# JoeyYoung/adapcc

Hardware: AMD Instinct MI355X
Metric: gpt2_ddp_tokens_per_sec (higher is better)
Workload: dtype bf16; 1 GPU; model=gpt2-small-124M, global_batch=128, seq_len=1024, parallelism=dp1, bucket_cap_mb=100, hipgraph=True, precision=bf16, transport=native

## Files before the change

### adapcc_amd/models/gpt2.py

```python

from __future__ import annotations

import math
from dataclasses import dataclass

import torch
import torch.nn as nn
import torch.nn.functional as F

from ..ops.fused import FusedLayerNorm


@dataclass
class GPT2Config:
    vocab_size: int = 50257
    n_positions: int = 1024
    n_embd: int = 768
    n_layer: int = 12
    n_head: int = 12
    dropout: float = 0.0

    @classmethod
    def small(cls) -> "GPT2Config":
        return cls()

    @classmethod
    def tiny(cls) -> "GPT2Config":
        return cls(vocab_size=2048, n_positions=256, n_embd=128, n_layer=2,
                   n_head=4)

    @classmethod
    def medium(cls) -> "GPT2Config":
        return cls(n_embd=1024, n_layer=24, n_head=16)


class CausalSelfAttention(nn.Module):
    def __init__(self, cfg: GPT2Config):
        super().__init__()
        assert cfg.n_embd % cfg.n_head == 0
        self.n_head = cfg.n_head
        self.c_attn = nn.Linear(cfg.n_embd, 3 * cfg.n_embd)
        self.c_proj = nn.Linear(cfg.n_embd, cfg.n_embd)
        self.dropout = cfg.dropout

    def forward(self, x: torch.Tensor) -> torch.Tensor:
        B, T, C = x.shape
        qkv = self.c_attn(x)
        q, k, v = qkv.split(C, dim=2)
        hd = C // self.n_head
        q = q.view(B, T, self.n_head, hd).transpose(1, 2)
        k = k.view(B, T, self.n_head, hd).transpose(1, 2)
        v = v.view(B, T, self.n_head, hd).transpose(1, 2)
        from ..ops.attention import flash_attention

        y = flash_attention(
            q, k, v, causal=True,
            dropout_p=self.dropout if self.training else 0.0,
        )
        y = y.transpose(1, 2).contiguous().view(B, T, C)
        return self.c_proj(y)


class MLP(nn.Module):
    def __init__(self, cfg: GPT2Config):
        super().__init__()
        self.c_fc = nn.Linear(cfg.n_embd, 4 * cfg.n_embd)
        self.c_proj = nn.Linear(4 * cfg.n_embd, cfg.n_embd)

    def forward(self, x: torch.Tensor) -> torch.Tensor:
        from ..ops.fused import fused_gelu

        return self.c_proj(fused_gelu(self.c_fc(x)))


class Block(nn.Module):
    def __init__(self, cfg: GPT2Config):
        super().__init__()
        self.ln_1 = FusedLayerNorm(cfg.n_embd)
        self.attn = CausalSelfAttention(cfg)
        self.ln_2 = FusedLayerNorm(cfg.n_embd)
        self.mlp = MLP(cfg)

    def forward(self, x: torch.Tensor) -> torch.Tensor:
        x = x + self.attn(self.ln_1(x))
        x = x + self.mlp(self.ln_2(x))
        return x


class GPT2(nn.Module):
    def __init__(self, cfg: GPT2Config):
        super().__init__()
        self.cfg = cfg
        self.wte = nn.Embedding(cfg.vocab_size, cfg.n_embd)
        self.wpe = nn.Embedding(cfg.n_positions, cfg.n_embd)
        self.drop = nn.Dropout(cfg.dropout)
        self.h = nn.ModuleList(Block(cfg) for _ in range(cfg.n_layer))
        self.ln_f = FusedLayerNorm(cfg.n_embd)
        self.lm_head = nn.Linear(cfg.n_embd, cfg.vocab_size, bias=False)
        self.lm_head.weight = self.wte.weight
        self.apply(self._init)
        for name, p in self.named_parameters():
            if name.endswith("c_proj.weight"):
                nn.init.normal_(p, mean=0.0,
                                std=0.02 / math.sqrt(2 * cfg.n_layer))

    @staticmethod
    def _init(m: nn.Module) -> None:
        if isinstance(m, nn.Linear):
            nn.init.normal_(m.weight, mean=0.0, std=0.02)
            if m.bias is not None:
                nn.init.zeros_(m.bias)
        elif isinstance(m, nn.Embedding):
            nn.init.normal_(m.weight, mean=0.0, std=0.02)

    def num_params(self, non_embedding: bool = True) -> int:
        n = sum(p.numel() for p in self.parameters())
        if non_embedding:
            n -= self.wpe.weight.numel()
        return n

    def forward(self, idx: torch.Tensor, targets: torch.Tensor = None):
        B, T = idx.shape
        pos = torch.arange(T, device=idx.device)
        x = self.drop(self.wte(idx) + self.wpe(pos))
        for block in self.h:
            x = block(x)
        x = self.ln_f(x)
        logits = self.lm_head(x)
        loss = None
        if targets is not None:
            from ..ops.fused import fused_cross_entropy

            loss = fused_cross_entropy(
                logits.view(-1, logits.size(-1)), targets.view(-1)
            )
        return logits, loss
```

### adapcc_amd/ops/attention.py

```python

from __future__ import annotations

import math

import torch

from .fused import _core

__all__ = ["flash_attention", "fa_supported"]


def _strides3(t: torch.Tensor):
    return [t.stride(0), t.stride(1), t.stride(2)]


def _row_ok(t: torch.Tensor) -> bool:
    if t.stride(3) != 1:
        return False
    if t.data_ptr() % 16 != 0:
        return False
    return all(s % 8 == 0 for s in _strides3(t))


def fa_supported(q: torch.Tensor, k: torch.Tensor, v: torch.Tensor,
                 causal: bool, dropout_p: float) -> bool:
    if not (causal and dropout_p == 0.0):
        return False
    if not (q.is_cuda and q.dtype == torch.bfloat16):
        return False
    if q.dim() != 4 or q.shape != k.shape or q.shape != v.shape:
        return False
    B, H, S, D = q.shape
    if D != 64 or S % 128 != 0 or S < 128:
        return False
    if not (_row_ok(q) and _row_ok(k) and _row_ok(v)):
        return False
    return bool(_core())


class _FlashAttnFn(torch.autograd.Function):
    @staticmethod
    def forward(ctx, q, k, v, scale):
        c = _core()
        B, H, S, D = q.shape
        o = torch.empty((B, H, S, D), dtype=q.dtype, device=q.device)
        lse = torch.empty((B, H, S), dtype=torch.float32, device=q.device)
        strides = _strides3(q) + _strides3(k) + _strides3(v) + _strides3(o)
        stream = torch.cuda.current_stream(q.device).cuda_stream
        c.fa_fwd(q.data_ptr(), k.data_ptr(), v.data_ptr(), o.data_ptr(),
                 lse.data_ptr(), B, H, S, strides, scale, stream)
        ctx.save_for_backward(q, k, v, o, lse)
        ctx.scale = scale
        return o

    @staticmethod
    def backward(ctx, dout):
        c = _core()
        q, k, v, o, lse = ctx.saved_tensors
        B, H, S, D = q.shape
        do = dout.contiguous()
        delta = (do.float() * o.float()).sum(-1)
        dq = torch.empty((B, H, S, D), dtype=q.dtype, device=q.device)
        dk = torch.empty_like(dq)
        dv = torch.empty_like(dq)
        strides = (_strides3(q) + _strides3(k) + _strides3(v) +
                   _strides3(do) + _strides3(dq) + _strides3(dk) +
                   _strides3(dv))
        stream = torch.cuda.current_stream(q.device).cuda_stream
        c.fa_bwd(q.data_ptr(), k.data_ptr(), v.data_ptr(), do.data_ptr(),
                 lse.data_ptr(), delta.data_ptr(), dq.data_ptr(),
                 dk.data_ptr(), dv.data_ptr(), B, H, S, strides, ctx.scale,
                 stream)
        return dq, dk, dv, None


def flash_attention(q: torch.Tensor, k: torch.Tensor, v: torch.Tensor,
                    causal: bool = True, dropout_p: float = 0.0,
                    scale: float = None) -> torch.Tensor:
    if fa_supported(q, k, v, causal, dropout_p):
        s = scale if scale is not None else 1.0 / math.sqrt(q.shape[-1])
        return _FlashAttnFn.apply(q, k, v, s)
    return torch.nn.functional.scaled_dot_product_attention(
        q, k, v, is_causal=causal, dropout_p=dropout_p, scale=scale)
```

### adapcc_amd/ops/csrc/attn.hip

```cpp

#include <hip/hip_runtime.h>
#include <hip/hip_bf16.h>

#include <cstdint>
#include <stdexcept>
#include <string>

namespace adapcc {

namespace {

typedef __attribute__((ext_vector_type(8))) __bf16 bf16x8;
typedef __attribute__((ext_vector_type(4))) __bf16 bf16x4;
typedef __attribute__((ext_vector_type(16))) float f32x16;

constexpr int kQT = 128;
constexpr float kNegBig = -3.0e38f;
constexpr float kLog2e = 1.4426950408889634f;
constexpr float kLn2 = 0.6931471805599453f;

__device__ __forceinline__ f32x16 mfma(bf16x8 a, bf16x8 b, f32x16 c) {
  return __builtin_amdgcn_mfma_f32_32x32x16_bf16(a, b, c, 0, 0, 0);
}

// ... 91 lines not shown

  const int qb = qt * kQT + wave * 32;
  const int qrow = qb + (lane & 31);

  bf16x8 qf[4];
#pragma unroll
  for (int c = 0; c < 4; ++c)
    qf[c] = *reinterpret_cast<const bf16x8*>(
        qg + (long)qrow * p.qs.ss + c * 16 + hi * 8);

  f32x16 acc0 = {}, acc1 = {};
  float m = kNegBig, ssum = 0.f;
  const float c1 = p.scale * kLog2e;
  float mc = m * c1;
  const float thr = 8.0f / p.scale;

  const int srow = threadIdx.x >> 3;
  const int scol = (threadIdx.x & 7) * 8;
  const int n64 = (qt + 1) * (kQT / 64);

  {
    *reinterpret_cast<uint4*>(kimg(0) + row_img_byte(srow, scol)) =
        *reinterpret_cast<const uint4*>(kg + (long)srow * p.ks.ss + scol);
    *reinterpret_cast<uint4*>(kimg(0) + 4096 + row_img_byte(srow, scol)) =
        *reinterpret_cast<const uint4*>(kg + (long)(srow + 32) * p.ks.ss +
                                        scol);
    *reinterpret_cast<uint4*>(vimg(0) + row_img_byte(srow, scol)) =
        *reinterpret_cast<const uint4*>(vg + (long)srow * p.vs.ss + scol);
    *reinterpret_cast<uint4*>(vimg(0) + 4096 + row_img_byte(srow, scol)) =
        *reinterpret_cast<const uint4*>(vg + (long)(srow + 32) * p.vs.ss +
                                        scol);
  }
  __syncthreads();

  int cur = 0;
  for (int t = 0; t < n64; ++t) {
    uint4 nk0, nk1, nv0, nv1;
    const bool pref = t + 1 < n64;
    if (pref) {
      const long kb0 = (long)(t + 1) * 64 + srow;
      nk0 = *reinterpret_cast<const uint4*>(kg + kb0 * p.ks.ss + scol);
      nk1 = *reinterpret_cast<const uint4*>(kg + (kb0 + 32) * p.ks.ss + scol);
      nv0 = *reinterpret_cast<const uint4*>(vg + kb0 * p.vs.ss + scol);
      nv1 = *reinterpret_cast<const uint4*>(vg + (kb0 + 32) * p.vs.ss + scol);
    }

#pragma unroll
    for (int half = 0; half < 2; ++half) {
      const int kbase = t * 64 + half * 32;
      if (kbase > qb + 31) break;
      const char* ki = kimg(cur) + half * 4096;
      const char* vi = vimg(cur) + half * 4096;

      f32x16 s = {};
      __builtin_amdgcn_s_setprio(1);
#pragma unroll
      for (int c = 0; c < 4; ++c)
        s = mfma(read_row_frag(ki, lane, c), qf[c], s);
      __builtin_amdgcn_s_setprio(0);

      float pv[16];
      float tmax = kNegBig;
      if (kbase + 31 > qb) {
#pragma unroll
        for (int r = 0; r < 16; ++r) {
          const int kglob = kbase + crow(r, hi);
          pv[r] = (kglob > qrow) ? kNegBig : s[r];
          tmax = fmaxf(tmax, pv[r]);
        }
      } else {
#pragma unroll
        for (int r = 0; r < 16; ++r) {
          pv[r] = s[r];
          tmax = fmaxf(tmax, pv[r]);
        }
      }
      tmax = fmaxf(tmax, __shfl_xor(tmax, 32, 64));
      if (!__all(tmax <= m + thr)) {
        const float mnew = fmaxf(m, tmax);
        const float alpha = __builtin_amdgcn_exp2f((m - mnew) * c1);
        m = mnew;
        mc = m * c1;
        ssum *= alpha;
#pragma unroll
        for (int r = 0; r < 16; ++r) {
          acc0[r] *= alpha;
          acc1[r] *= alpha;
        }
      }

      float psum = 0.f;
#pragma unroll
      for (int r = 0; r < 16; ++r) {
        pv[r] = __builtin_amdgcn_exp2f(__builtin_fmaf(pv[r], c1, -mc));
        psum += pv[r];
      }
      ssum += psum;

      const bf16x8 p0 = pack_frag(&pv[0]);
      const bf16x8 p1 = pack_frag(&pv[8]);

      __builtin_amdgcn_s_setprio(1);
      acc0 = mfma(read_tr_frag(vi, lane, 0, 0), p0, acc0);
      acc0 = mfma(read_tr_frag(vi, lane, 1, 0), p1, acc0);
      acc1 = mfma(read_tr_frag(vi, lane, 0, 1), p0, acc1);
      acc1 = mfma(read_tr_frag(vi, lane, 1, 1), p1, acc1);
      __builtin_amdgcn_s_setprio(0);
    }

    if (pref) {
      *reinterpret_cast<uint4*>(kimg(cur ^ 1) + row_img_byte(srow, scol)) =
          nk0;
      *reinterpret_cast<uint4*>(kimg(cur ^ 1) + 4096 +
                                row_img_byte(srow, scol)) = nk1;
      *reinterpret_cast<uint4*>(vimg(cur ^ 1) + row_img_byte(srow, scol)) =
          nv0;
      *reinterpret_cast<uint4*>(vimg(cur ^ 1) + 4096 +
                                row_img_byte(srow, scol)) = nv1;
    }
    __syncthreads();
    cur ^= 1;
  }

  const float stot = ssum + __shfl_xor(ssum, 32, 64);
  const float inv = 1.f / stot;
  if ((lane >> 5) == 0)
    lseg[qrow] = p.scale * m + __builtin_amdgcn_logf(stot) * kLn2;

  __bf16* orow = og + (long)qrow * p.os.ss;
#pragma unroll
  for (int db = 0; db < 2; ++db) {
    const f32x16& a = db ? acc1 : acc0;
#pragma unroll
    for (int mq = 0; mq < 4; ++mq) {
      const int d0 = db * 32 + 8 * mq + 4 * hi;
      unsigned lo, hi2;
      asm("v_cvt_pk_bf16_f32 %0, %2, %3\n\t"
          "v_cvt_pk_bf16_f32 %1, %4, %5"
          : "=&v"(lo), "=&v"(hi2)
          : "v"(a[4 * mq] * inv), "v"(a[4 * mq + 1] * inv),
            "v"(a[4 * mq + 2] * inv), "v"(a[4 * mq + 3] * inv));
      uint2 st = {lo, hi2};
      *reinterpret_cast<uint2*>(orow + d0) = st;
    }
  }
}
#undef kimg
#undef vimg

struct FaBwdParams {
  const __bf16* q;
  const __bf16* k;
  const __bf16* v;
  const __bf16* dout;
  const float* lse;
  const float* delta;
  __bf16* dq;
  __bf16* dk;
  __bf16* dv;
  TStride qs, ks, vs, dos_, dqs, dks, dvs;
  int H, S;
  float scale;
};

__global__ __launch_bounds__(256, 3) void fa_bwd_dq_kernel(FaBwdParams p) {
  __shared__ __attribute__((aligned(16))) char smem[4 * 8192];
#define kimg(i) (smem + (i) * 8192)
#define vimg(i) (smem + 16384 + (i) * 8192)

  const int lane = threadIdx.x & 63;
  const int wave = threadIdx.x >> 6;
  const int hi = lane >> 5;
  const int qt = blockIdx.x;
  const int bh = blockIdx.y;
  const int b = bh / p.H, h = bh % p.H;

  const __bf16* qg = p.q + (long)b * p.qs.sb + (long)h * p.qs.sh;
  const __bf16* kg = p.k + (long)b * p.ks.sb + (long)h * p.ks.sh;
  const __bf16* vg = p.v + (long)b * p.vs.sb + (long)h * p.vs.sh;
  const __bf16* dog = p.dout + (long)b * p.dos_.sb + (long)h * p.dos_.sh;
  __bf16* dqg = p.dq + (long)b * p.dqs.sb + (long)h * p.dqs.sh;

  const int qb = qt * kQT + wave * 32;
  const int qrow = qb + (lane & 31);

  bf16x8 qf[4], dof[4];
#pragma unroll
  for (int c = 0; c < 4; ++c) {
    qf[c] = *reinterpret_cast<const bf16x8*>(
        qg + (long)qrow * p.qs.ss + c * 16 + hi * 8);
    dof[c] = *reinterpret_cast<const bf16x8*>(
        dog + (long)qrow * p.dos_.ss + c * 16 + hi * 8);
  }
  const float lse2 = p.lse[(long)bh * p.S + qrow] * kLog2e;
  const float dvq = p.delta[(long)bh * p.S + qrow];
  const float c1 = p.scale * kLog2e;

  f32x16 dacc0 = {}, dacc1 = {};

  const int srow = threadIdx.x >> 3;
  const int scol = (threadIdx.x & 7) * 8;
  const int n64 = (qt + 1) * (kQT / 64);
  {
    *reinterpret_cast<uint4*>(kimg(0) + row_img_byte(srow, scol)) =
        *reinterpret_cast<const uint4*>(kg + (long)srow * p.ks.ss + scol);
    *reinterpret_cast<uint4*>(kimg(0) + 4096 + row_img_byte(srow, scol)) =
        *reinterpret_cast<const uint4*>(kg + (long)(srow + 32) * p.ks.ss +
                                        scol);
    *reinterpret_cast<uint4*>(vimg(0) + row_img_byte(srow, scol)) =
        *reinterpret_cast<const uint4*>(vg + (long)srow * p.vs.ss + scol);
    *reinterpret_cast<uint4*>(vimg(0) + 4096 + row_img_byte(srow, scol)) =
        *reinterpret_cast<const uint4*>(vg + (long)(srow + 32) * p.vs.ss +
                                        scol);
  }
  __syncthreads();

  int cur = 0;
  for (int t = 0; t < n64; ++t) {
    uint4 nk0, nk1, nv0, nv1;
    const bool pref = t + 1 < n64;
    if (pref) {
      const long kb0 = (long)(t + 1) * 64 + srow;
      nk0 = *reinterpret_cast<const uint4*>(kg + kb0 * p.ks.ss + scol);
      nk1 = *reinterpret_cast<const uint4*>(kg + (kb0 + 32) * p.ks.ss + scol);
      nv0 = *reinterpret_cast<const uint4*>(vg + kb0 * p.vs.ss + scol);
      nv1 = *reinterpret_cast<const uint4*>(vg + (kb0 + 32) * p.vs.ss + scol);
    }

#pragma unroll
    for (int half = 0; half < 2; ++half) {
      const int kbase = t * 64 + half * 32;
      if (kbase > qb + 31) break;
      const char* ki = kimg(cur) + half * 4096;
      const char* vi = vimg(cur) + half * 4096;

      f32x16 s = {}, dp = {};
      __builtin_amdgcn_s_setprio(1);
#pragma unroll
      for (int c = 0; c < 4; ++c) {
        s = mfma(read_row_frag(ki, lane, c), qf[c], s);
        dp = mfma(read_row_frag(vi, lane, c), dof[c], dp);
      }
      __builtin_amdgcn_s_setprio(0);

      float ds[16];
      if (kbase + 31 > qb) {
#pragma unroll
        for (int r = 0; r < 16; ++r) {
          const int kglob = kbase + crow(r, hi);
          const float pe =
              (kglob > qrow)
                  ? 0.f
                  : __builtin_amdgcn_exp2f(__builtin_fmaf(s[r], c1, -lse2));
          ds[r] = pe * (dp[r] - dvq) * p.scale;
        }
      } else {
#pragma unroll
        for (int r = 0; r < 16; ++r) {
          const float pe =
              __builtin_amdgcn_exp2f(__builtin_fmaf(s[r], c1, -lse2));
          ds[r] = pe * (dp[r] - dvq) * p.scale;
        }
      }
      const bf16x8 d0 = pack_frag(&ds[0]);
      const bf16x8 d1 = pack_frag(&ds[8]);
      __builtin_amdgcn_s_setprio(1);
      dacc0 = mfma(read_tr_frag(ki, lane, 0, 0), d0, dacc0);
      dacc0 = mfma(read_tr_frag(ki, lane, 1, 0), d1, dacc0);
      dacc1 = mfma(read_tr_frag(ki, lane, 0, 1), d0, dacc1);
      dacc1 = mfma(read_tr_frag(ki, lane, 1, 1), d1, dacc1);
      __builtin_amdgcn_s_setprio(0);
    }

    if (pref) {
      *reinterpret_cast<uint4*>(kimg(cur ^ 1) + row_img_byte(srow, scol)) =
          nk0;
      *reinterpret_cast<uint4*>(kimg(cur ^ 1) + 4096 +
                                row_img_byte(srow, scol)) = nk1;
      *reinterpret_cast<uint4*>(vimg(cur ^ 1) + row_img_byte(srow, scol)) =
          nv0;
      *reinterpret_cast<uint4*>(vimg(cur ^ 1) + 4096 +
                                row_img_byte(srow, scol)) = nv1;
    }
    __syncthreads();
    cur ^= 1;
  }

  __bf16* drow = dqg + (long)qrow * p.dqs.ss;
#pragma unroll
  for (int db = 0; db < 2; ++db) {
    const f32x16& a = db ? dacc1 : dacc0;
#pragma unroll
    for (int mq = 0; mq < 4; ++mq) {
      const int d0 = db * 32 + 8 * mq + 4 * hi;
      unsigned lo, hi2;
      asm("v_cvt_pk_bf16_f32 %0, %2, %3\n\t"
          "v_cvt_pk_bf16_f32 %1, %4, %5"
          : "=&v"(lo), "=&v"(hi2)
          : "v"(a[4 * mq]), "v"(a[4 * mq + 1]), "v"(a[4 * mq + 2]),
            "v"(a[4 * mq + 3]));
      uint2 st = {lo, hi2};
      *reinterpret_cast<uint2*>(drow + d0) = st;
    }
  }
}
#undef kimg
#undef vimg


__global__ __launch_bounds__(256, 2) void fa_bwd_dkv_kernel(FaBwdParams p) {
  __shared__ __attribute__((aligned(16))) char smem[4 * 8192 + 1024];
#define qimg(i) (smem + (i) * 8192)
#define doimg(i) (smem + 16384 + (i) * 8192)
#define lsetile (reinterpret_cast<float*>(smem + 32768))
#define dtile (reinterpret_cast<float*>(smem + 32768 + 512))

  const int lane = threadIdx.x & 63;
  const int wave = threadIdx.x >> 6;
  const int hi = lane >> 5;
  const int kt = blockIdx.x;
  const int bh = blockIdx.y;
  const int b = bh / p.H, h = bh % p.H;

  const __bf16* qg = p.q + (long)b * p.qs.sb + (long)h * p.qs.sh;
  const __bf16* kg = p.k + (long)b * p.ks.sb + (long)h * p.ks.sh;
  const __bf16* vg = p.v + (long)b * p.vs.sb + (long)h * p.vs.sh;
  const __bf16* dog = p.dout + (long)b * p.dos_.sb + (long)h * p.dos_.sh;
  __bf16* dkg = p.dk + (long)b * p.dks.sb + (long)h * p.dks.sh;
  __bf16* dvg = p.dv + (long)b * p.dvs.sb + (long)h * p.dvs.sh;
  const float* lseg = p.lse + (long)bh * p.S;
  const float* deltag = p.delta + (long)bh * p.S;

  const int kbb = kt * kQT + wave * 32;
  const int krow = kbb + (lane & 31);

  bf16x8 kf[4], vf[4];
#pragma unroll
  for (int c = 0; c < 4; ++c) {
    kf[c] = *reinterpret_cast<const bf16x8*>(
        kg + (long)krow * p.ks.ss + c * 16 + hi * 8);
    vf[c] = *reinterpret_cast<const bf16x8*>(
        vg + (long)krow * p.vs.ss + c * 16 + hi * 8);
  }

  const float c1 = p.scale * kLog2e;
  f32x16 dvacc0 = {}, dvacc1 = {}, dkacc0 = {}, dkacc1 = {};

  const int srow = threadIdx.x >> 3;
// ... 78 lines not shown
          const float pe = __builtin_amdgcn_exp2f(
              __builtin_fmaf(sacc[r], c1, -lsec[crow(r, hi)]));
          pv[r] = pe;
          ds[r] = pe * (dp[r] - dc[crow(r, hi)]) * p.scale;
        }
      }
      const bf16x8 p0 = pack_frag(&pv[0]);
      const bf16x8 p1 = pack_frag(&pv[8]);
      __builtin_amdgcn_s_setprio(1);
      dvacc0 = mfma(p0, read_tr_frag(di, lane, 0, 0), dvacc0);
      dvacc0 = mfma(p1, read_tr_frag(di, lane, 1, 0), dvacc0);
      dvacc1 = mfma(p0, read_tr_frag(di, lane, 0, 1), dvacc1);
      dvacc1 = mfma(p1, read_tr_frag(di, lane, 1, 1), dvacc1);
      __builtin_amdgcn_s_setprio(0);
      const bf16x8 e0 = pack_frag(&ds[0]);
      const bf16x8 e1 = pack_frag(&ds[8]);
      __builtin_amdgcn_s_setprio(1);
      dkacc0 = mfma(e0, read_tr_frag(qi, lane, 0, 0), dkacc0);
      dkacc0 = mfma(e1, read_tr_frag(qi, lane, 1, 0), dkacc0);
      dkacc1 = mfma(e0, read_tr_frag(qi, lane, 0, 1), dkacc1);
      dkacc1 = mfma(e1, read_tr_frag(qi, lane, 1, 1), dkacc1);
      __builtin_amdgcn_s_setprio(0);
    }

    if (pref) {
      *reinterpret_cast<uint4*>(qimg(cur ^ 1) + row_img_byte(srow, scol)) =
          nq0;
      *reinterpret_cast<uint4*>(qimg(cur ^ 1) + 4096 +
                                row_img_byte(srow, scol)) = nq1;
      *reinterpret_cast<uint4*>(doimg(cur ^ 1) + row_img_byte(srow, scol)) =
          nd0;
      *reinterpret_cast<uint4*>(doimg(cur ^ 1) + 4096 +
                                row_img_byte(srow, scol)) = nd1;
      if (threadIdx.x < 64) {
        lsetile[((cur ^ 1) ? 64 : 0) + threadIdx.x] = nlse;
        dtile[((cur ^ 1) ? 64 : 0) + threadIdx.x] = ndel;
      }
    }
    __syncthreads();
    cur ^= 1;
  }

  __syncthreads();
  float* scratch = reinterpret_cast<float*>(smem) + wave * 2048;
#pragma unroll
  for (int t = 0; t < 2; ++t) {
    const f32x16& a0 = t ? dkacc0 : dvacc0;
    const f32x16& a1 = t ? dkacc1 : dvacc1;
#pragma unroll
    for (int r = 0; r < 16; ++r) {
      scratch[crow(r, hi) * 64 + (lane & 31)] = a0[r];
      scratch[crow(r, hi) * 64 + 32 + (lane & 31)] = a1[r];
    }
    __builtin_amdgcn_s_waitcnt(0);
    __bf16* outg = (t ? dkg : dvg);
    const TStride& os = t ? p.dks : p.dvs;
    const int row = lane >> 1;
    const int dhalf = (lane & 1) * 32;
#pragma unroll
    for (int mq = 0; mq < 8; ++mq) {
      const float* src = scratch + row * 64 + dhalf + mq * 4;
      unsigned lo, hi2;
      asm("v_cvt_pk_bf16_f32 %0, %2, %3\n\t"
          "v_cvt_pk_bf16_f32 %1, %4, %5"
          : "=&v"(lo), "=&v"(hi2)
          : "v"(src[0]), "v"(src[1]), "v"(src[2]), "v"(src[3]));
      uint2 st = {lo, hi2};
      *reinterpret_cast<uint2*>(outg + (long)(kbb + row) * os.ss + dhalf +
                                mq * 4) = st;
    }
    __syncthreads();
  }
}
#undef qimg
#undef doimg
#undef lsetile
#undef dtile

__global__ void tr_probe_kernel(float* out, int kb, int db) {
  __shared__ __attribute__((aligned(16))) char img[4096];
  const int lane = threadIdx.x & 63;
  for (int i = threadIdx.x; i < 2048; i += 64) {
    const int k = i / 64, d = i % 64;
    *reinterpret_cast<__bf16*>(img + row_img_byte(k, d)) =
        (__bf16)(float)(k * 64 + d);
  }
  __syncthreads();
  bf16x8 f = read_tr_frag(img, lane, kb, db);
  union {
    bf16x8 v;
    __bf16 e[8];
  } u;
  u.v = f;
#pragma unroll
  for (int e = 0; e < 8; ++e) out[lane * 8 + e] = (float)u.e[e];
}

__global__ void pack_probe_kernel(float* out) {
  const int lane = threadIdx.x & 63;
  float p[8];
#pragma unroll
  for (int r = 0; r < 8; ++r) p[r] = (float)(lane * 100 + r);
  bf16x8 f = pack_frag(p);
  union {
    bf16x8 v;
    __bf16 e[8];
  } u;
  u.v = f;
#pragma unroll
  for (int e = 0; e < 8; ++e) out[lane * 8 + e] = (float)u.e[e];
}

__global__ void mfma_probe_kernel(const __bf16* a, const __bf16* b, float* c) {
  const int lane = threadIdx.x & 63;
  union {
    __bf16 e[8];
    bf16x8 f;
  } af, bf;
#pragma unroll
  for (int e = 0; e < 8; ++e) {
    af.e[e] = a[(lane % 32) * 16 + 8 * (lane / 32) + e];
    bf.e[e] = b[(8 * (lane / 32) + e) * 32 + (lane % 32)];
  }
  f32x16 acc = {};
  acc = mfma(af.f, bf.f, acc);
#pragma unroll
  for (int r = 0; r < 16; ++r)
    c[crow(r, lane >> 5) * 32 + (lane % 32)] = acc[r];
}

}

void fa_forward(const void* q, const void* k, const void* v, void* o,
                float* lse, int B, int H, int S, const long* strides,
                float scale, hipStream_t stream) {
  if (S % kQT != 0) throw std::runtime_error("fa_forward: S % 128 != 0");
  FaParams p;
  p.q = (const __bf16*)q;
  p.k = (const __bf16*)k;
  p.v = (const __bf16*)v;
  p.o = (__bf16*)o;
  p.lse = lse;
  p.qs = {strides[0], strides[1], strides[2]};
  p.ks = {strides[3], strides[4], strides[5]};
  p.vs = {strides[6], strides[7], strides[8]};
  p.os = {strides[9], strides[10], strides[11]};
  p.H = H;
  p.S = S;
  p.scale = scale;
  dim3 grid(S / kQT, B * H);
  hipLaunchKernelGGL(fa_fwd_kernel, grid, dim3(256), 0, stream, p);
}

void fa_backward(const void* q, const void* k, const void* v, const void* do_,
                 const float* lse, const float* delta, void* dq, void* dk,
                 void* dv, int B, int H, int S, const long* strides,
                 float scale, hipStream_t stream) {
  if (S % kQT != 0) throw std::runtime_error("fa_backward: S % 128 != 0");
  FaBwdParams p;
  p.q = (const __bf16*)q;
  p.k = (const __bf16*)k;
  p.v = (const __bf16*)v;
  p.dout = (const __bf16*)do_;
  p.lse = lse;
  p.delta = delta;
  p.dq = (__bf16*)dq;
  p.dk = (__bf16*)dk;
  p.dv = (__bf16*)dv;
  p.qs = {strides[0], strides[1], strides[2]};
  p.ks = {strides[3], strides[4], strides[5]};
  p.vs = {strides[6], strides[7], strides[8]};
  p.dos_ = {strides[9], strides[10], strides[11]};
  p.dqs = {strides[12], strides[13], strides[14]};
  p.dks = {strides[15], strides[16], strides[17]};
  p.dvs = {strides[18], strides[19], strides[20]};
  p.H = H;
  p.S = S;
  p.scale = scale;
  dim3 grid(S / kQT, B * H);
  hipLaunchKernelGGL(fa_bwd_dq_kernel, grid, dim3(256), 0, stream, p);
  hipLaunchKernelGGL(fa_bwd_dkv_kernel, grid, dim3(256), 0, stream, p);
}

void mfma_probe(const void* a, const void* b, float* c, hipStream_t stream) {
  hipLaunchKernelGGL(mfma_probe_kernel, dim3(1), dim3(64), 0, stream,
                     (const __bf16*)a, (const __bf16*)b, c);
}

void tr_probe(float* out, int kb, int db, hipStream_t stream) {
  hipLaunchKernelGGL(tr_probe_kernel, dim3(1), dim3(64), 0, stream, out, kb,
                     db);
}

void pack_probe(float* out, hipStream_t stream) {
  hipLaunchKernelGGL(pack_probe_kernel, dim3(1), dim3(64), 0, stream, out);
}

}
```

### adapcc_amd/ops/csrc/bindings.hip

```cpp

#include <pybind11/pybind11.h>
#include <pybind11/stl.h>

#include "common.h"
#include "engine.h"
#include "plan.h"

namespace py = pybind11;
using adapcc::Engine;

static py::dict plan_to_dict(const adapcc::PlanData& p) {
  py::list cs, rs, bs;
  for (const auto& u : p.cunits) {
    py::dict d;
    d["tree"] = u.tree; d["chunk"] = u.chunk;
    d["offset"] = u.offset_elems; d["count"] = u.count_elems;
    d["flag_space"] = (int)u.flag_space;
    py::list nl;
    for (int i = 0; i < u.nnotify; ++i) nl.append(u.notify_rank[i]);
    d["notify_to"] = nl;
    cs.append(d);
  }
  for (const auto& u : p.runits) {
    py::dict d;
    d["tree"] = u.tree; d["chunk"] = u.chunk;
    d["offset"] = u.offset_elems; d["count"] = u.count_elems;
    py::list srcs;
    for (int s = 0; s < u.nsrc; ++s)
      srcs.append(py::make_tuple(u.src_rank[s], (int)u.src_kind[s]));
    d["srcs"] = srcs;
    d["include_self"] = (bool)u.include_self;
    d["notify"] = (bool)u.notify_parent; d["consumer"] = u.parent_rank;
    d["is_root"] = (bool)u.is_root;
    py::list kids;
    for (int c = 0; c < u.nchildren; ++c) kids.append(u.child_rank[c]);
    d["publish_to"] = kids;
    rs.append(d);
  }
  for (const auto& u : p.bunits) {
    py::dict d;
    d["tree"] = u.tree; d["chunk"] = u.chunk;
    d["src_offset"] = u.src_offset_elems; d["dst_offset"] = u.dst_offset_elems;
    d["count"] = u.count_elems;
    d["parent"] = u.parent_rank; d["parent_kind"] = (int)u.parent_kind;
    d["forward"] = (bool)u.forward;
    py::list kids;
    for (int c = 0; c < u.nchildren; ++c) kids.append(u.child_rank[c]);
    d["publish_to"] = kids;
    bs.append(d);
  }
  py::dict out;
  out["copy"] = cs;
  out["reduce"] = rs;
  out["bcast"] = bs;
  out["chunk_elems"] = p.chunk_elems;
  return out;
}

namespace adapcc {
void launch_local_reduce(Dtype dt, void* dst, const void* const* srcs_dev,
                         int nsrc, long count, RedOp op, float scale,
                         hipStream_t stream);
bool ln_supported_api(long cols, int dtype);
void ln_forward(int dtype, const void* x, const void* w, const void* b,
                void* y, float* mean, float* rstd, long rows, long cols,
                float eps, hipStream_t stream);
void ln_backward(int dtype, const void* dy, const void* x, const void* w,
                 const float* mean, const float* rstd, void* dx,
                 float* ws_gamma, float* ws_beta, long rows, long cols,
                 int nblocks, hipStream_t stream);
void ce_forward(int dtype, const void* logits, const void* targets,
                float* loss, float* lse, long rows, long cols,
                long ignore_index, hipStream_t stream);
void ce_backward(int dtype, const void* logits, const void* targets,
                 const float* lse, const float* gscale, void* dlogits,
                 long rows, long cols, long ignore_index, hipStream_t stream);
void fa_forward(const void* q, const void* k, const void* v, void* o,
                float* lse, int B, int H, int S, const long* strides,
                float scale, hipStream_t stream);
void fa_backward(const void* q, const void* k, const void* v, const void* do_,
                 const float* lse, const float* delta, void* dq, void* dk,
                 void* dv, int B, int H, int S, const long* strides,
                 float scale, hipStream_t stream);
void mfma_probe(const void* a, const void* b, float* c, hipStream_t stream);
void gelu_forward(int dtype, const void* x, void* y, long n,
                  hipStream_t stream);
void gelu_backward(int dtype, const void* x, const void* dy, void* dx, long n,
                   hipStream_t stream);
void tr_probe(float* out, int kb, int db, hipStream_t stream);
void pack_probe(float* out, hipStream_t stream);
}

PYBIND11_MODULE(_core, m) {
  m.doc() = "adapcc_amd native engine (MI355X / gfx950)";

  m.def("local_reduce",
        [](uintptr_t dst, const std::vector<uintptr_t>& srcs, long count,
           int dtype, int op, float scale, uintptr_t stream) {
          if (srcs.empty()) throw std::runtime_error("no sources");
          void** d_srcs = nullptr;
          hipError_t e = hipMalloc(&d_srcs, srcs.size() * sizeof(void*));
          if (e != hipSuccess) throw std::runtime_error(hipGetErrorString(e));
          e = hipMemcpy(d_srcs, srcs.data(), srcs.size() * sizeof(void*),
                        hipMemcpyHostToDevice);
          if (e != hipSuccess) throw std::runtime_error(hipGetErrorString(e));
          adapcc::launch_local_reduce(
              (adapcc::Dtype)dtype, reinterpret_cast<void*>(dst),
              (const void* const*)d_srcs, (int)srcs.size(), count,
              (adapcc::RedOp)op, scale, reinterpret_cast<hipStream_t>(stream));
          e = hipGetLastError();
          if (e != hipSuccess) throw std::runtime_error(hipGetErrorString(e));
          e = hipStreamSynchronize(reinterpret_cast<hipStream_t>(stream));
          (void)hipFree(d_srcs);
          if (e != hipSuccess) throw std::runtime_error(hipGetErrorString(e));
        },
        py::arg("dst"), py::arg("srcs"), py::arg("count"), py::arg("dtype"),
        py::arg("op"), py::arg("scale") = 1.0f, py::arg("stream") = 0);

  m.def("ln_supported", &adapcc::ln_supported_api, py::arg("cols"),
        py::arg("dtype"));
  m.def("ln_fwd",
        [](int dtype, uintptr_t x, uintptr_t w, uintptr_t b, uintptr_t y,
           uintptr_t mean, uintptr_t rstd, long rows, long cols, float eps,
           uintptr_t stream) {
          adapcc::ln_forward(dtype, (const void*)x, (const void*)w,
                             (const void*)b, (void*)y, (float*)mean,
                             (float*)rstd, rows, cols, eps,
                             reinterpret_cast<hipStream_t>(stream));
          hipError_t e = hipGetLastError();
          if (e != hipSuccess) throw std::runtime_error(hipGetErrorString(e));
        });
  m.def("ln_bwd",
        [](int dtype, uintptr_t dy, uintptr_t x, uintptr_t w, uintptr_t mean,
           uintptr_t rstd, uintptr_t dx, uintptr_t wsg, uintptr_t wsb,
           long rows, long cols, int nblocks, uintptr_t stream) {
          adapcc::ln_backward(dtype, (const void*)dy, (const void*)x,
                              (const void*)w, (const float*)mean,
                              (const float*)rstd, (void*)dx, (float*)wsg,
                              (float*)wsb, rows, cols, nblocks,
                              reinterpret_cast<hipStream_t>(stream));
          hipError_t e = hipGetLastError();
          if (e != hipSuccess) throw std::runtime_error(hipGetErrorString(e));
        });

  m.def("ce_fwd",
        [](int dtype, uintptr_t logits, uintptr_t targets, uintptr_t loss,
           uintptr_t lse, long rows, long cols, long ignore_index,
           uintptr_t stream) {
          adapcc::ce_forward(dtype, (const void*)logits,
                             (const void*)targets, (float*)loss, (float*)lse,
                             rows, cols, ignore_index,
                             reinterpret_cast<hipStream_t>(stream));
          hipError_t e = hipGetLastError();
          if (e != hipSuccess) throw std::runtime_error(hipGetErrorString(e));
        });
  m.def("ce_bwd",
        [](int dtype, uintptr_t logits, uintptr_t targets, uintptr_t lse,
           uintptr_t gscale, uintptr_t dlogits, long rows, long cols,
           long ignore_index, uintptr_t stream) {
          adapcc::ce_backward(dtype, (const void*)logits,
                              (const void*)targets, (const float*)lse,
                              (const float*)gscale, (void*)dlogits, rows,
                              cols, ignore_index,
                              reinterpret_cast<hipStream_t>(stream));
          hipError_t e = hipGetLastError();
          if (e != hipSuccess) throw std::runtime_error(hipGetErrorString(e));
        });

  m.def("fa_fwd",
        [](uintptr_t q, uintptr_t k, uintptr_t v, uintptr_t o, uintptr_t lse,
           int B, int H, int S, const std::vector<long>& strides, float scale,
           uintptr_t stream) {
          if (strides.size() != 12)
            throw std::runtime_error("fa_fwd: need 12 strides");
          adapcc::fa_forward((const void*)q, (const void*)k, (const void*)v,
                             (void*)o, (float*)lse, B, H, S, strides.data(),
                             scale, reinterpret_cast<hipStream_t>(stream));
          hipError_t e = hipGetLastError();
          if (e != hipSuccess) throw std::runtime_error(hipGetErrorString(e));
        });
  m.def("fa_bwd",
        [](uintptr_t q, uintptr_t k, uintptr_t v, uintptr_t dout,
           uintptr_t lse, uintptr_t delta, uintptr_t dq, uintptr_t dk,
           uintptr_t dv, int B, int H, int S, const std::vector<long>& strides,
           float scale, uintptr_t stream) {
          if (strides.size() != 21)
            throw std::runtime_error("fa_bwd: need 21 strides");
          adapcc::fa_backward((const void*)q, (const void*)k, (const void*)v,
                              (const void*)dout, (const float*)lse,
                              (const float*)delta, (void*)dq, (void*)dk,
                              (void*)dv, B, H, S, strides.data(), scale,
                              reinterpret_cast<hipStream_t>(stream));
          hipError_t e = hipGetLastError();
          if (e != hipSuccess) throw std::runtime_error(hipGetErrorString(e));
        });
  m.def("mfma_probe",
        [](uintptr_t a, uintptr_t b, uintptr_t c, uintptr_t stream) {
          adapcc::mfma_probe((const void*)a, (const void*)b, (float*)c,
                             reinterpret_cast<hipStream_t>(stream));
          hipError_t e = hipGetLastError();
          if (e != hipSuccess) throw std::runtime_error(hipGetErrorString(e));
        });

  m.def("gelu_fwd",
        [](int dtype, uintptr_t x, uintptr_t y, long n, uintptr_t stream) {
          adapcc::gelu_forward(dtype, (const void*)x, (void*)y, n,
                               reinterpret_cast<hipStream_t>(stream));
          hipError_t e = hipGetLastError();
          if (e != hipSuccess) throw std::runtime_error(hipGetErrorString(e));
        });
  m.def("gelu_bwd",
        [](int dtype, uintptr_t x, uintptr_t dy, uintptr_t dx, long n,
           uintptr_t stream) {
          adapcc::gelu_backward(dtype, (const void*)x, (const void*)dy,
                                (void*)dx, n,
                                reinterpret_cast<hipStream_t>(stream));
          hipError_t e = hipGetLastError();
          if (e != hipSuccess) throw std::runtime_error(hipGetErrorString(e));
        });

  m.def("tr_probe",
        [](uintptr_t out, int kb, int db, uintptr_t stream) {
          adapcc::tr_probe((float*)out, kb, db,
                           reinterpret_cast<hipStream_t>(stream));
          hipError_t e = hipGetLastError();
          if (e != hipSuccess) throw std::runtime_error(hipGetErrorString(e));
        });
  m.def("pack_probe",
        [](uintptr_t out, uintptr_t stream) {
          adapcc::pack_probe((float*)out,
                             reinterpret_cast<hipStream_t>(stream));
          hipError_t e = hipGetLastError();
          if (e != hipSuccess) throw std::runtime_error(hipGetErrorString(e));
        });

  m.def("compute_plan",
        [](const std::vector<std::vector<int>>& parents, int rank,
           long total_elems, int esize, long chunk_bytes,
           const std::vector<int>& active,
           const std::vector<double>& slice_weights) {
          auto shape = adapcc::TreeShape::derive(parents);
          uint64_t mask = 0;
          for (int r : active) mask |= (1ull << r);
          if (active.empty()) mask = (1ull << shape.world) - 1;
          return plan_to_dict(adapcc::build_plan(shape, rank, total_elems,
                                                 esize, chunk_bytes, mask,
                                                 slice_weights));
        },
        py::arg("parents"), py::arg("rank"), py::arg("total_elems"),
        py::arg("esize"), py::arg("chunk_bytes"),
        py::arg("active") = std::vector<int>{},
        py::arg("slice_weights") = std::vector<double>{});

  m.def("compute_primitive_plan",
        [](const std::string& prim, int world, int rank, long elems, int esize,
           long chunk_bytes, int root,
           const std::vector<std::vector<int>>& parents,
           const std::vector<int>& active,
           const std::vector<double>& slice_weights) {
          uint64_t mask = 0;
          for (int r : active) mask |= (1ull << r);
          if (active.empty()) mask = (1ull << world) - 1;
          adapcc::PlanData pd;
          if (prim == "reduce") {
            auto shape = parents.empty() ? adapcc::star_shape(world)
                                         : adapcc::TreeShape::derive(parents);
            pd = adapcc::build_reduce_plan(shape, rank, root, elems, esize,
                                           chunk_bytes, mask, slice_weights);
          } else if (prim == "broadcast") {
            pd = adapcc::build_broadcast_plan(world, rank, root, elems, esize,
                                              chunk_bytes);
          } else if (prim == "allgather") {
            pd = adapcc::build_allgather_plan(world, rank, elems, esize,
                                              chunk_bytes);
          } else if (prim == "reducescatter") {
            pd = adapcc::build_reducescatter_plan(world, rank, elems, esize,
                                                  chunk_bytes, mask);
          } else if (prim == "alltoall") {
            pd = adapcc::build_alltoall_plan(world, rank, elems, esize,
                                             chunk_bytes);
          } else {
            throw std::runtime_error("unknown primitive " + prim);
          }
          return plan_to_dict(pd);
        },
        py::arg("prim"), py::arg("world"), py::arg("rank"), py::arg("elems"),
        py::arg("esize"), py::arg("chunk_bytes"), py::arg("root") = 0,
        py::arg("parents") = std::vector<std::vector<int>>{},
        py::arg("active") = std::vector<int>{},
        py::arg("slice_weights") = std::vector<double>{});

  py::class_<Engine>(m, "Engine")
      .def(py::init<int, int, int, size_t, double>(), py::arg("rank"),
           py::arg("world"), py::arg("device"), py::arg("cap_bytes"),
           py::arg("timeout_ms"))
      .def("ipc_handle",
           [](Engine& e) { return py::bytes(e.ipc_handle()); })
      .def("connect",
           [](Engine& e, const std::vector<py::bytes>& handles,
              const std::vector<int>& peer_devices) {
             std::vector<std::string> hs;
             hs.reserve(handles.size());
             for (const auto& h : handles) hs.push_back(std::string(h));
             e.connect(hs, peer_devices);
           },
           py::arg("handles"), py::arg("peer_devices") = std::vector<int>{})
      .def("set_strategy", &Engine::set_strategy, py::arg("parents"),
           py::arg("chunk_bytes"),
           py::arg("slice_weights") = std::vector<double>{})
      .def("connect_local", &Engine::connect_local, py::arg("peer_addrs"))
      .def("region_addr", &Engine::region_addr)
      .def("allreduce",
           [](Engine& e, uintptr_t data_ptr, long numel, int dtype, int op,
              const std::vector<int>& active, bool average,
              uintptr_t stream) {
             e.allreduce(reinterpret_cast<void*>(data_ptr), numel, dtype, op,
                         active, average, reinterpret_cast<void*>(stream));
           },
           py::arg("data_ptr"), py::arg("numel"), py::arg("dtype"),
           py::arg("op"), py::arg("active"), py::arg("average"),
           py::arg("stream"))
      .def("reduce",
           [](Engine& e, uintptr_t data_ptr, long numel, int dtype, int op,
              int root, const std::vector<int>& active, uintptr_t stream) {
             e.reduce(reinterpret_cast<void*>(data_ptr), numel, dtype, op,
                      root, active, reinterpret_cast<void*>(stream));
           },
           py::arg("data_ptr"), py::arg("numel"), py::arg("dtype"),
           py::arg("op"), py::arg("root"), py::arg("active"),
           py::arg("stream"))
      .def("broadcast",
           [](Engine& e, uintptr_t data_ptr, long numel, int dtype, int root,
              uintptr_t stream) {
             e.broadcast(reinterpret_cast<void*>(data_ptr), numel, dtype, root,
                         reinterpret_cast<void*>(stream));
           },
           py::arg("data_ptr"), py::arg("numel"), py::arg("dtype"),
           py::arg("root"), py::arg("stream"))
      .def("all_gather",
           [](Engine& e, uintptr_t in_ptr, uintptr_t out_ptr, long in_elems,
              int dtype, uintptr_t stream) {
             e.all_gather(reinterpret_cast<const void*>(in_ptr),
                          reinterpret_cast<void*>(out_ptr), in_elems, dtype,
                          reinterpret_cast<void*>(stream));
           },
// ... 43 lines not shown
```

Before: 699,500 tokens/s.

## Fuse QKV head split/merge into flash attention and compute delta in-kernel

Attention now takes the packed QKV tensor directly and passes strided head views to the kernels. Output is written straight into (B,T,C) layout and gradients straight into a packed dQKV buffer, which removes the transpose/contiguous copies and the autograd split/cat. The backward dq kernel also computes delta = rowsum(dO*O) itself and writes it out, replacing the separate PyTorch float elementwise-and-reduce pass. The risk is that other backward kernels (dk/dv) read delta, so it must be written before they run, which depends on launch order.

```diff
diff --git a/adapcc_amd/models/gpt2.py b/adapcc_amd/models/gpt2.py
--- a/adapcc_amd/models/gpt2.py
+++ b/adapcc_amd/models/gpt2.py
@@ -44,21 +44,12 @@
         self.dropout = cfg.dropout
 
     def forward(self, x: torch.Tensor) -> torch.Tensor:
-        B, T, C = x.shape
-        qkv = self.c_attn(x)
-        q, k, v = qkv.split(C, dim=2)
-        hd = C // self.n_head
-        q = q.view(B, T, self.n_head, hd).transpose(1, 2)
-        k = k.view(B, T, self.n_head, hd).transpose(1, 2)
-        v = v.view(B, T, self.n_head, hd).transpose(1, 2)
-        from ..ops.attention import flash_attention
+        from ..ops import attention
 
-        y = flash_attention(
-            q, k, v, causal=True,
+        return self.c_proj(attention.flash_attention_qkv(
+            self.c_attn(x), self.n_head,
             dropout_p=self.dropout if self.training else 0.0,
-        )
-        y = y.transpose(1, 2).contiguous().view(B, T, C)
-        return self.c_proj(y)
+        ))
 
 
 class MLP(nn.Module):
diff --git a/adapcc_amd/ops/attention.py b/adapcc_amd/ops/attention.py
--- a/adapcc_amd/ops/attention.py
+++ b/adapcc_amd/ops/attention.py
@@ -7,7 +7,8 @@
 
 from .fused import _core
 
-__all__ = ["flash_attention", "fa_supported"]
+__all__ = ["flash_attention", "flash_attention_qkv", "fa_supported",
+           "fa_qkv_supported"]
 
 
 def _strides3(t: torch.Tensor):
@@ -38,40 +39,83 @@
     return bool(_core())
 
 
+def _launch_fwd(q, k, v, o, lse, scale):
+    B, H, S, _ = q.shape
+    strides = _strides3(q) + _strides3(k) + _strides3(v) + _strides3(o)
+    stream = torch.cuda.current_stream(q.device).cuda_stream
+    _core().fa_fwd(q.data_ptr(), k.data_ptr(), v.data_ptr(), o.data_ptr(),
+                   lse.data_ptr(), B, H, S, strides, scale, stream)
+
+
+def _launch_bwd(q, k, v, o, dout, lse, dq, dk, dv, scale):
+    B, H, S, _ = q.shape
+    do = dout if _row_ok(dout) else dout.contiguous()
+    delta = torch.empty((B, H, S), dtype=torch.float32, device=q.device)
+    strides = (_strides3(q) + _strides3(k) + _strides3(v) + _strides3(o) +
+               _strides3(do) + _strides3(dq) + _strides3(dk) +
+               _strides3(dv))
+    stream = torch.cuda.current_stream(q.device).cuda_stream
+    _core().fa_bwd(q.data_ptr(), k.data_ptr(), v.data_ptr(), o.data_ptr(),
+                   do.data_ptr(), lse.data_ptr(), delta.data_ptr(),
+                   dq.data_ptr(), dk.data_ptr(), dv.data_ptr(), B, H, S,
+                   strides, scale, stream)
+
+
 class _FlashAttnFn(torch.autograd.Function):
     @staticmethod
     def forward(ctx, q, k, v, scale):
-        c = _core()
         B, H, S, D = q.shape
-        o = torch.empty((B, H, S, D), dtype=q.dtype, device=q.device)
+        o = torch.empty((B, S, H, D), dtype=q.dtype,
+                        device=q.device).transpose(1, 2)
         lse = torch.empty((B, H, S), dtype=torch.float32, device=q.device)
-        strides = _strides3(q) + _strides3(k) + _strides3(v) + _strides3(o)
-        stream = torch.cuda.current_stream(q.device).cuda_stream
-        c.fa_fwd(q.data_ptr(), k.data_ptr(), v.data_ptr(), o.data_ptr(),
-                 lse.data_ptr(), B, H, S, strides, scale, stream)
+        _launch_fwd(q, k, v, o, lse, scale)
         ctx.save_for_backward(q, k, v, o, lse)
         ctx.scale = scale
         return o
 
     @staticmethod
     def backward(ctx, dout):
-        c = _core()
         q, k, v, o, lse = ctx.saved_tensors
         B, H, S, D = q.shape
-        do = dout.contiguous()
-        delta = (do.float() * o.float()).sum(-1)
         dq = torch.empty((B, H, S, D), dtype=q.dtype, device=q.device)
         dk = torch.empty_like(dq)
         dv = torch.empty_like(dq)
-        strides = (_strides3(q) + _strides3(k) + _strides3(v) +
-                   _strides3(do) + _strides3(dq) + _strides3(dk) +
-                   _strides3(dv))
-        stream = torch.cuda.current_stream(q.device).cuda_stream
-        c.fa_bwd(q.data_ptr(), k.data_ptr(), v.data_ptr(), do.data_ptr(),
-                 lse.data_ptr(), delta.data_ptr(), dq.data_ptr(),
-                 dk.data_ptr(), dv.data_ptr(), B, H, S, strides, ctx.scale,
-                 stream)
+        _launch_bwd(q, k, v, o, dout, lse, dq, dk, dv, ctx.scale)
         return dq, dk, dv, None
+
+
+def _heads(t: torch.Tensor, n_head: int) -> torch.Tensor:
+    B, T, C = t.shape
+    return t.view(B, T, n_head, C // n_head).transpose(1, 2)
+
+
+class _FlashAttnQkvFn(torch.autograd.Function):
+
+    @staticmethod
+    def forward(ctx, qkv, n_head, scale):
+        B, T, C3 = qkv.shape
+        C = C3 // 3
+        q, k, v = (_heads(t, n_head) for t in qkv.split(C, dim=2))
+        y = torch.empty((B, T, C), dtype=qkv.dtype, device=qkv.device)
+        lse = torch.empty((B, n_head, T), dtype=torch.float32,
+                          device=qkv.device)
+        _launch_fwd(q, k, v, _heads(y, n_head), lse, scale)
+        ctx.save_for_backward(qkv, y, lse)
+        ctx.n_head = n_head
+        ctx.scale = scale
+        return y
+
+    @staticmethod
+    def backward(ctx, dy):
+        qkv, y, lse = ctx.saved_tensors
+        H = ctx.n_head
+        C = y.shape[2]
+        q, k, v = (_heads(t, H) for t in qkv.split(C, dim=2))
+        dqkv = torch.empty_like(qkv)
+        dq, dk, dv = (_heads(t, H) for t in dqkv.split(C, dim=2))
+        _launch_bwd(q, k, v, _heads(y, H), _heads(dy, H), lse, dq, dk, dv,
+                    ctx.scale)
+        return dqkv, None, None
 
 
 def flash_attention(q: torch.Tensor, k: torch.Tensor, v: torch.Tensor,
@@ -82,3 +126,36 @@
         return _FlashAttnFn.apply(q, k, v, s)
     return torch.nn.functional.scaled_dot_product_attention(
         q, k, v, is_causal=causal, dropout_p=dropout_p, scale=scale)
+
+
+def _attention_qkv_composed(qkv: torch.Tensor, n_head: int,
+                            dropout_p: float = 0.0) -> torch.Tensor:
+    B, T, C3 = qkv.shape
+    C = C3 // 3
+    q, k, v = (_heads(t, n_head) for t in qkv.split(C, dim=2))
+    y = flash_attention(q, k, v, causal=True, dropout_p=dropout_p)
+    return y.transpose(1, 2).contiguous().view(B, T, C)
+
+
+def fa_qkv_supported(qkv: torch.Tensor, n_head: int,
+                     dropout_p: float) -> bool:
+    if dropout_p != 0.0:
+        return False
+    if not (qkv.is_cuda and qkv.dtype == torch.bfloat16 and qkv.dim() == 3):
+        return False
+    B, T, C3 = qkv.shape
+    if C3 % (3 * n_head) != 0 or C3 // (3 * n_head) != 64:
+        return False
+    if T % 128 != 0 or T < 128 or B < 1:
+        return False
+    if not qkv.is_contiguous() or qkv.data_ptr() % 16 != 0:
+        return False
+    return bool(_core())
+
+
+def flash_attention_qkv(qkv: torch.Tensor, n_head: int,
+                        dropout_p: float = 0.0) -> torch.Tensor:
+    if fa_qkv_supported(qkv, n_head, dropout_p):
+        scale = 1.0 / math.sqrt(qkv.shape[2] // (3 * n_head))
+        return _FlashAttnQkvFn.apply(qkv, n_head, scale)
+    return _attention_qkv_composed(qkv, n_head, dropout_p)
diff --git a/adapcc_amd/ops/csrc/attn.hip b/adapcc_amd/ops/csrc/attn.hip
--- a/adapcc_amd/ops/csrc/attn.hip
+++ b/adapcc_amd/ops/csrc/attn.hip
@@ -267,16 +267,35 @@
   const __bf16* q;
   const __bf16* k;
   const __bf16* v;
+  const __bf16* o;
   const __bf16* dout;
   const float* lse;
-  const float* delta;
+  float* delta;
   __bf16* dq;
   __bf16* dk;
   __bf16* dv;
-  TStride qs, ks, vs, dos_, dqs, dks, dvs;
+  TStride qs, ks, vs, os, dos_, dqs, dks, dvs;
   int H, S;
   float scale;
 };
+
+__device__ __forceinline__ float dot8_tree(bf16x8 a, bf16x8 b) {
+  union {
+    bf16x8 f;
+    unsigned u[4];
+  } x, y;
+  x.f = a;
+  y.f = b;
+  float pr[4];
+#pragma unroll
+  for (int i = 0; i < 4; ++i) {
+    const float ev = __builtin_fmaf(__uint_as_float(x.u[i] << 16),
+                                    __uint_as_float(y.u[i] << 16), 0.f);
+    pr[i] = __builtin_fmaf(__uint_as_float(x.u[i] & 0xffff0000u),
+                           __uint_as_float(y.u[i] & 0xffff0000u), ev);
+  }
+  return (pr[0] + pr[1]) + (pr[2] + pr[3]);
+}
 
 __global__ __launch_bounds__(256, 3) void fa_bwd_dq_kernel(FaBwdParams p) {
   __shared__ __attribute__((aligned(16))) char smem[4 * 8192];
@@ -294,21 +313,30 @@
   const __bf16* kg = p.k + (long)b * p.ks.sb + (long)h * p.ks.sh;
   const __bf16* vg = p.v + (long)b * p.vs.sb + (long)h * p.vs.sh;
   const __bf16* dog = p.dout + (long)b * p.dos_.sb + (long)h * p.dos_.sh;
+  const __bf16* og = p.o + (long)b * p.os.sb + (long)h * p.os.sh;
   __bf16* dqg = p.dq + (long)b * p.dqs.sb + (long)h * p.dqs.sh;
 
   const int qb = qt * kQT + wave * 32;
   const int qrow = qb + (lane & 31);
 
   bf16x8 qf[4], dof[4];
+  float n16[4];
 #pragma unroll
   for (int c = 0; c < 4; ++c) {
+    dof[c] = *reinterpret_cast<const bf16x8*>(
+        dog + (long)qrow * p.dos_.ss + c * 16 + hi * 8);
+    const float n8 = dot8_tree(
+        dof[c], *reinterpret_cast<const bf16x8*>(
+                    og + (long)qrow * p.os.ss + c * 16 + hi * 8));
+    n16[c] = n8 + __shfl_xor(n8, 32, 64);
+  }
+#pragma unroll
+  for (int c = 0; c < 4; ++c)
     qf[c] = *reinterpret_cast<const bf16x8*>(
         qg + (long)qrow * p.qs.ss + c * 16 + hi * 8);
-    dof[c] = *reinterpret_cast<const bf16x8*>(
-        dog + (long)qrow * p.dos_.ss + c * 16 + hi * 8);
-  }
   const float lse2 = p.lse[(long)bh * p.S + qrow] * kLog2e;
-  const float dvq = p.delta[(long)bh * p.S + qrow];
+  const float dvq = (n16[0] + n16[1]) + (n16[2] + n16[3]);
+  if (hi == 0) p.delta[(long)bh * p.S + qrow] = dvq;
   const float c1 = p.scale * kLog2e;
 
   f32x16 dacc0 = {}, dacc1 = {};
@@ -693,15 +721,16 @@
   hipLaunchKernelGGL(fa_fwd_kernel, grid, dim3(256), 0, stream, p);
 }
 
-void fa_backward(const void* q, const void* k, const void* v, const void* do_,
-                 const float* lse, const float* delta, void* dq, void* dk,
-                 void* dv, int B, int H, int S, const long* strides,
+void fa_backward(const void* q, const void* k, const void* v, const void* o,
+                 const void* do_, const float* lse, float* delta, void* dq,
+                 void* dk, void* dv, int B, int H, int S, const long* strides,
                  float scale, hipStream_t stream) {
   if (S % kQT != 0) throw std::runtime_error("fa_backward: S % 128 != 0");
   FaBwdParams p;
   p.q = (const __bf16*)q;
   p.k = (const __bf16*)k;
   p.v = (const __bf16*)v;
+  p.o = (const __bf16*)o;
   p.dout = (const __bf16*)do_;
   p.lse = lse;
   p.delta = delta;
@@ -711,10 +740,11 @@
   p.qs = {strides[0], strides[1], strides[2]};
   p.ks = {strides[3], strides[4], strides[5]};
   p.vs = {strides[6], strides[7], strides[8]};
-  p.dos_ = {strides[9], strides[10], strides[11]};
-  p.dqs = {strides[12], strides[13], strides[14]};
-  p.dks = {strides[15], strides[16], strides[17]};
-  p.dvs = {strides[18], strides[19], strides[20]};
+  p.os = {strides[9], strides[10], strides[11]};
+  p.dos_ = {strides[12], strides[13], strides[14]};
+  p.dqs = {strides[15], strides[16], strides[17]};
+  p.dks = {strides[18], strides[19], strides[20]};
+  p.dvs = {strides[21], strides[22], strides[23]};
   p.H = H;
   p.S = S;
   p.scale = scale;
diff --git a/adapcc_amd/ops/csrc/bindings.hip b/adapcc_amd/ops/csrc/bindings.hip
--- a/adapcc_amd/ops/csrc/bindings.hip
+++ b/adapcc_amd/ops/csrc/bindings.hip
@@ -78,9 +78,9 @@
 void fa_forward(const void* q, const void* k, const void* v, void* o,
                 float* lse, int B, int H, int S, const long* strides,
                 float scale, hipStream_t stream);
-void fa_backward(const void* q, const void* k, const void* v, const void* do_,
-                 const float* lse, const float* delta, void* dq, void* dk,
-                 void* dv, int B, int H, int S, const long* strides,
+void fa_backward(const void* q, const void* k, const void* v, const void* o,
+                 const void* do_, const float* lse, float* delta, void* dq,
+                 void* dk, void* dv, int B, int H, int S, const long* strides,
                  float scale, hipStream_t stream);
 void mfma_probe(const void* a, const void* b, float* c, hipStream_t stream);
 void gelu_forward(int dtype, const void* x, void* y, long n,
@@ -180,17 +180,17 @@
           if (e != hipSuccess) throw std::runtime_error(hipGetErrorString(e));
         });
   m.def("fa_bwd",
-        [](uintptr_t q, uintptr_t k, uintptr_t v, uintptr_t dout,
+        [](uintptr_t q, uintptr_t k, uintptr_t v, uintptr_t o, uintptr_t dout,
            uintptr_t lse, uintptr_t delta, uintptr_t dq, uintptr_t dk,
            uintptr_t dv, int B, int H, int S, const std::vector<long>& strides,
            float scale, uintptr_t stream) {
-          if (strides.size() != 21)
-            throw std::runtime_error("fa_bwd: need 21 strides");
+          if (strides.size() != 24)
+            throw std::runtime_error("fa_bwd: need 24 strides");
           adapcc::fa_backward((const void*)q, (const void*)k, (const void*)v,
-                              (const void*)dout, (const float*)lse,
-                              (const float*)delta, (void*)dq, (void*)dk,
-                              (void*)dv, B, H, S, strides.data(), scale,
-                              reinterpret_cast<hipStream_t>(stream));
+                              (const void*)o, (const void*)dout,
+                              (const float*)lse, (float*)delta, (void*)dq,
+                              (void*)dk, (void*)dv, B, H, S, strides.data(),
+                              scale, reinterpret_cast<hipStream_t>(stream));
           hipError_t e = hipGetLastError();
           if (e != hipSuccess) throw std::runtime_error(hipGetErrorString(e));
         });
```

Result: faster. 787,300 tokens/s, median of 6 (+12.6%).
